# KyungMinJin/OTPose

Hardware: AMD Instinct MI355X
Metric: frames/sec at 384x288, 5-frame window, batch 16; heatmap max-abs delta vs ref (higher is better)
Workload: dtype f32 storage+accumulate / f16x3 split products; 1 GPU; BASELINE configs[1]: batch 16 x 5-frame x 384x288, HRNet-W48 + DCN warp + ConvVideoTransformer, fp32 forward (eval), seeded synthetic weights; clips_per_gpu=16, parallelism=dp1, outputs_finite=True

## Files before the change

include/otpose_hip.h:

```cpp
#ifndef OTPOSE_HIP_H
#define OTPOSE_HIP_H

#include <stddef.h>

#ifdef __cplusplus
extern "C" {
#endif

#define OTP_OK 0
#define OTP_ERR_BAD_ARG (-1)
#define OTP_ERR_UNSUPPORTED (-2)
#define OTP_ERR_LAUNCH (-3)
#define OTP_ERR_WORKSPACE (-4)

#define OTP_DTYPE_F32 0
#define OTP_DTYPE_F16 1
#define OTP_DTYPE_BF16 2
#define OTP_DTYPE_F64 3
#define OTP_DTYPE_I64 4

#define OTP_ACT_NONE 0
#define OTP_ACT_RELU 1
#define OTP_ACT_GELU 2

// ... 237 lines not shown
int otp_upsample_linear(const void* x, void* out, int B, int C, int T, int f, int out_ctot, int out_coff, void* stream);

int otp_mlp_fused_supported(int C, int HID, int T);
size_t otp_mlp_fused_weight_bytes(int C, int HID);
int otp_mlp_fused_pack(const void* w1, const void* b1, const void* w2, void* packed, int C, int HID, void* stream);
int otp_mlp_fused(const void* x, const void* packed, const void* scale, const void* shift, const void* res, void* out,
                  int B, int C, int HID, int T, void* stream);
int otp_ln_mlp_fused(const void* y, const void* ln_gamma, const void* ln_beta, float ln_eps, const void* packed,
                     const void* scale, const void* shift, void* out, int B, int C, int HID, int T, void* stream);

int otp_dense_x3_supported(int C, int T);
size_t otp_dense_x3_weight_bytes(int C);
int otp_dense_x3_pack(const void* w, const void* scale, const void* shift, void* packed, int C, void* stream);
int otp_dense_x3(const void* const* x, const void* const* packed, const void* const* res, void* const* out, int nprob, int B,
                 int C, int T, void* stream);
int otp_dense_x3_pack_bf16p(const void* w, const void* scale, const void* shift, void* packed, int C, void* stream);
int otp_dense_x3_bf16p(const void* const* x, const void* const* packed, const void* const* res, void* const* out, int nprob, int B,
                 int C, int T, void* stream);
int otp_qkv_front_x3(const void* x, const void* table, const void* packed_q, const void* packed_k, const void* packed_v,
                     void* q, void* k, void* v, int B, int C, int T, float eps, void* stream);

int otp_stem_conv_x3_supported(int B, int F, int H, int W, int Cout);
size_t otp_stem_conv_x3_weight_bytes(int Cout);
int otp_stem_conv_x3_pack(const void* w, const void* scale, const void* shift, void* packed, int Cout, void* stream);
int otp_stem_conv_x3(const void* in, const void* packed, void* out, int B, int F, int H, int W, int Cout, void* stream);

int otp_pointwise_x3_supported(int Cin, int Cout, int T);
size_t otp_pointwise_x3_weight_bytes(int Cin, int Cout);
int otp_pointwise_x3_pack(const void* w, const void* scale, const void* shift, void* packed, int Cin, int Cout, void* stream);
int otp_pointwise_x3(const void* x, const void* packed, const void* res, void* out, int B, int Cin, int Cout, int T, int x_ctot,
                     int x_coff, int res_ctot, int res_coff, int out_ctot, int out_coff, int relu, void* stream);
int otp_pointwise_x3_s8_supported(int Cin, int Cout, int T);
size_t otp_pointwise_x3_s8_weight_bytes(int Cin, int Cout);
int otp_pointwise_x3_s8_pack(const void* w, const void* scale, const void* shift, void* packed, int Cin, int Cout, void* stream);
int otp_pointwise_x3_s8(const void* x, const void* packed, void* out_s8, int B, int Cin, int Cout, int T, int x_ctot, int x_coff,
                        int relu, void* stream);
int otp_pointwise_x3_s8_res(const void* x, const void* packed, const void* res, void* out_s8, int B, int Cin, int Cout, int T,
                            int x_ctot, int x_coff, int r_ctot, int r_coff, int relu, void* stream);
int otp_pointwise_x3_pair_supported(int Cin, int Cmid, int Cout2, int T);
size_t otp_pointwise_x3_pair_weight_bytes(int Cin, int Cmid, int Cout2);
int otp_pointwise_x3_pair_pack(const void* w1, const void* scale1, const void* shift1, const void* w2, const void* scale2,
                               const void* shift2, void* packed, int Cin, int Cmid, int Cout2, void* stream);
int otp_pointwise_x3_pair(const void* x, const void* packed, const void* res, void* out, void* out_s8, int B, int Cin, int Cmid,
                          int Cout2, int T, int x_ctot, int x_coff, int res_ctot, int res_coff, int out_ctot, int out_coff,
                          int relu1, int relu2, void* stream);

int otp_mlp_x3_supported(int C, int HID, int T);
size_t otp_mlp_x3_weight_bytes(int C, int HID);
int otp_mlp_x3_pack(const void* w1, const void* b1, const void* w2, void* packed, int C, int HID, void* stream);
int otp_mlp_x3(const void* x, const void* packed, const void* scale, const void* shift, const void* res, void* out, int B,
               int C, int HID, int T, void* stream);
int otp_ln_mlp_x3(const void* y, const void* ln_gamma, const void* ln_beta, float ln_eps, const void* packed,
                  const void* scale, const void* shift, void* out, int B, int C, int HID, int T, void* stream);

int otp_flow_block_supported(int C, int hidden, int T);
size_t otp_flow_front_param_floats(int C);
size_t otp_flow_back_param_floats(int C, int hidden);
int otp_flow_front(const void* x, const void* params, void* q, void* k, void* v, int B, int C, int T, float eps, void* stream);
int otp_flow_back(const void* x, const void* att, const void* params, void* out, int B, int C, int hidden, int T, float eps,
                  void* stream);

int otp_dense_cc_supported(int C, int T);
size_t otp_dense_cc_weight_bytes(int C);
int otp_dense_cc_pack(const void* w, const void* scale, const void* shift, void* packed, int C, void* stream);
int otp_dense_cc(const void* const* x, const void* const* packed, const void* const* res, void* const* out, int nprob,
                 int B, int C, int T, void* stream);

size_t otp_qkv_front_table_bytes(int C);
int otp_qkv_front_pack_table(const void* dwq, const void* dwk, const void* dwv, const void* gq, const void* bq,
                             const void* gk, const void* bk, const void* gv, const void* bv, void* table, int C,
                             void* stream);
int otp_qkv_front(const void* x, const void* table, const void* packed_q, const void* packed_k, const void* packed_v,
                  void* q, void* k, void* v, int B, int C, int T, float eps, void* stream);

int otp_upsample_add(const void* low, const void* res, void* out, int N, int C, int Hl, int Wl, int f, int relu,
                     int low_ctot, int low_coff, int res_ctot, int res_coff, int out_ctot, int out_coff, void* stream);
int otp_upsample_add_multi(const void* const* lows, const int* factors, int nlow, const void* res, void* out, int N, int C,
                           int Hh, int Wh, int relu, int res_ctot, int res_coff, int out_ctot, int out_coff, void* stream);

int otp_chan_attn_set_split(int on);
int otp_chan_attn_splits(int BH, int T);
int otp_chan_attn_scores(const void* a, const void* b, void* slabs, int BH, int hs, int T, void* stream);
int otp_chan_attn_apply(const void* v, const void* M, void* out, int BH, int hs, int T, void* stream);
int otp_chan_attn_scores_bf16p(const void* a, const void* b, void* slabs, int BH, int hs, int T, void* stream);
int otp_chan_attn_apply_bf16p(const void* v, const void* M, void* out, int BH, int hs, int T, void* stream);
int otp_transpose_scale(const void* in, void* out, int batches, int R, int Cc, float scale, void* stream);
int otp_softmax_backward(const void* slabs, const void* P, void* dS, void* dST, void* PT, int BH, int hs, int NS,
                         void* stream);
int otp_softmax_backward_dropout(const void* slabs, const void* P, void* dS, void* dST, void* PT, int BH, int hs, int NS, float p,
                                 unsigned long long seed, void* stream);
int otp_ln_channel_backward(const void* x, const void* grad_y, const void* gamma, void* grad_x, void* dy_xhat, int B, int C,
                            int T, float eps, void* stream);
size_t otp_ln_channel_backward_workspace(int B, int C, int T);
int otp_ln_channel_backward_params(const void* x, const void* grad_y, const void* gamma, void* grad_x, void* grad_gamma,
                                   void* grad_beta, void* workspace, size_t workspace_bytes, int B, int C, int T, float eps,
                                   void* stream);
int otp_dwconv3_forward(const void* x, const void* w, void* y, int B, int C, int T, int stride, void* stream);
int otp_dwconv3_backward(const void* x, const void* w, const void* grad_y, void* grad_x, void* grad_w, int B, int C, int T,
                         int stride, void* stream);
int otp_gelu_forward(const void* x, void* y, size_t n, void* stream);
int otp_gelu_backward(const void* x, const void* grad_y, void* grad_x, size_t n, void* stream);
int otp_maxpool3s2_forward(const void* x, void* y, int rows, int T, void* stream);
int otp_maxpool3s2_backward(const void* x, const void* grad_y, void* grad_x, int rows, int T, void* stream);
int otp_upsample_linear_backward(const void* grad_out, void* grad_x, int B, int C, int T, int f, int out_ctot, int out_coff,
                                 void* stream);

int otp_upsample_add_backward(const void* grad_out, const void* out_relu, void* grad_res, void* grad_low, int planes, int Hl,
                              int Wl, int f, void* stream);

int otp_axpby(const void* x, void* y, float alpha, float beta, size_t n, void* stream);

int otp_heatmap_decode(const void* heatmaps, void* preds, void* maxvals, const void* center, const void* scale,
                       int N, int J, int H, int W, int refine, void* stream);

int otp_heatmap_flip_decode(const void* heatmaps, const int* perm, void* merged, void* preds, void* maxvals,
                            const void* center, const void* scale, int B, int J, int H, int W, int shift, void* stream);
int otp_clip_mirror_pair(const void* x, void* out, int B, int C, int H, int W, void* stream);

int otp_pck_accuracy(const void* pred_coords, const void* target_coords, void* acc, void* cnt, int N, int J, int H, int W,
                     float thr, void* stream);

size_t otp_grad_sumsq_scratch(void);
int otp_grad_sumsq(const void* grad, size_t n, void* acc_f64, void* stream);
int otp_adamw_step(void* param, const void* grad, void* exp_avg, void* exp_avg_sq, size_t n, float lr, float beta1,
                   float beta2, float eps, float weight_decay, int step, const void* gradnorm_sq_f64, float max_norm,
                   void* stream);
int otp_sgd_step(void* param, const void* grad, void* momentum_buf, size_t n, float lr, float momentum, float dampening,
                 float weight_decay, int nesterov, int first_step, const void* gradnorm_sq_f64, float max_norm, void* stream);

int otp_ema_update(void* ema, const void* src, size_t n, float decay, float one_minus_decay, void* stream);
size_t otp_ema_job_bytes(void);
int otp_ema_job(void* ema, const void* src, size_t count, int dtype, const void* prev_job_host, void* job_host);
int otp_ema_update_table(const void* jobs_device, int n_jobs, float decay, float one_minus_decay, void* stream);

int otp_frames_u8_to_clip(const void* frames_u8, void* out, int B, int F, int H, int W, float mean_r, float mean_g,
                          float mean_b, float std_r, float std_g, float std_b, void* stream);

int otp_crop_clips_u8(const void* pool_u8, int S, int Hp, int Wp, const void* frame_idx, const void* M, const void* flip,
                      void* out, int B, int F, int H, int W, float mean_r, float mean_g, float mean_b, float std_r,
                      float std_g, float std_b, void* stream);
int otp_crop_clips_blur_u8(const void* pool_u8, int S, int Hp, int Wp, const void* frame_idx, const void* M,
                           const void* flip, void* out, int B, int F, int H, int W, float mean_r, float mean_g,
                           float mean_b, float std_r, float std_g, float std_b, const void* blur, const void* blur_on,
                           void* stream);
int otp_crop_clips_pair_u8(const void* pool_u8, int S, int Hp, int Wp, const void* frame_idx, const void* M, void* out,
                           int B, int F, int H, int W, float mean_r, float mean_g, float mean_b, float std_r, float std_g,
                           float std_b, void* stream);
int otp_pose_plan(const void* boxes, const void* scores, const void* counts, const void* frame_number,
                  const void* num_frames, int S, int K, int detect_lo, int detect_hi, double min_score, double aspect_ratio,
                  double enlarge, int out_w, int out_h, int posetrack18, int max_persons, void* center, void* scale, void* M,
                  void* frame_idx, void* margin, void* box_score, void* person_slot, void* pr_off, void* total, void* stream);
int otp_pose_targets(const void* joints, const void* vis, const void* M, const void* gauss, void* target,
                     void* target_weight, int B, int J, int W, int H, int w, int h, int sigma3, void* stream);

size_t otp_loss_workspace(int B, int J);
int otp_loss_st_ohkw_grads(const void* s, const void* t, const void* g, const void* w, void* flags, void* result,
                           void* grad_s, void* grad_t, void* grad_g, void* workspace, size_t workspace_bytes, int B, int J,
                           int HW, int topk, int flags_given, void* stream);
int otp_loss_st_ohkw(const void* s, const void* t, const void* g, const void* w, void* flags,
                     void* result, void* grad_s, void* grad_t, void* workspace, size_t workspace_bytes,
                     int B, int J, int HW, int topk, int flags_given, void* stream);
int otp_loss_joints_mse(const void* o, const void* g, const void* w, void* result, void* grad_o, void* workspace,
                        size_t workspace_bytes, int B, int J, int HW, int topk, int ohkm, int effective_num_joints,
                        void* stream);


// ... 114 lines not shown
```

otpose_amd/csrc/transformer.hip:

```cpp
#include "x3.h"
#include <cstdlib>
#include <type_traits>

namespace {

template <int CREG>
__global__ __launch_bounds__(256) void ln_channel_kernel(const float* __restrict__ x, const float* __restrict__ gamma,
                                                          const float* __restrict__ beta, float* __restrict__ y,
                                                          int C, int T, float eps) {
    const int t = blockIdx.x * blockDim.x + threadIdx.x;
    if (t >= T) return;
    const size_t base = (size_t)blockIdx.y * C * T + t;
    const float inv_c = 1.f / (float)C;
    if (CREG > 0) {
        float v[CREG > 0 ? CREG : 1];
        float s = 0.f;
#pragma unroll
        for (int c = 0; c < CREG; ++c) {
            v[c] = c < C ? x[base + (size_t)c * T] : 0.f;
            s += v[c];
        }
        const float mu = s * inv_c;
        float q = 0.f;
#pragma unroll
// ... 429 lines not shown
    const float* vb = v + (size_t)bh * hs * T;
    const float* pb = P + (size_t)bh * HSP * HSP;
    {
        constexpr int NP4 = (HSP * HSP / 4 + 255) / 256, NV4 = (HSP * (TT / 4) + 255) / 256;
        const bool vecv = (T & 3) == 0 && (reinterpret_cast<uintptr_t>(v) & 15) == 0;
        otp_f32x4 rp[NP4], rv[NV4];
#pragma unroll
        for (int j = 0; j < NP4; ++j) {
            const int idx = tid + j * 256;
            rp[j] = idx < HSP * HSP / 4 ? reinterpret_cast<const otp_f32x4*>(pb)[idx] : (otp_f32x4){0.f, 0.f, 0.f, 0.f};
        }
#pragma unroll
        for (int j = 0; j < NV4; ++j) {
            const int idx = tid + j * 256;
            const int row = idx / (TT / 4), t = t0 + 4 * (idx - row * (TT / 4));
            otp_f32x4 a = {0.f, 0.f, 0.f, 0.f};
            if (row < hs && idx < HSP * (TT / 4)) {
                const float* vp = vb + (size_t)row * T + t;
                if (vecv && t + 3 < T) {
                    a = *reinterpret_cast<const otp_f32x4*>(vp);
                } else {
#pragma unroll
                    for (int e = 0; e < 4; ++e)
                        if (t + e < T) a[e] = vp[e];
                }
            }
            rv[j] = a;
        }
#pragma unroll
        for (int j = 0; j < NP4; ++j) {
            const int idx = tid + j * 256;
            if (idx < HSP * HSP / 4) {
                const int i = (4 * idx) / HSP, jj = 4 * idx - i * HSP;
#pragma unroll
                for (int e = 0; e < 4; ++e) pl[i * PS + jj + e] = rp[j][e];
            }
        }
#pragma unroll
        for (int j = 0; j < NV4; ++j) {
            const int idx = tid + j * 256;
            if (idx < HSP * (TT / 4)) {
                const int row = idx / (TT / 4), tt = 4 * (idx - row * (TT / 4));
                *reinterpret_cast<otp_f32x4*>(vl + row * VS + tt) = rv[j];
            }
        }
    }
    __syncthreads();
    const int r16 = lane & 15, kk = lane >> 4;
    otp_f32x4 acc[TB][NB];
#pragma unroll
    for (int tb = 0; tb < TB; ++tb)
#pragma unroll
        for (int ib = 0; ib < NB; ++ib) acc[tb][ib] = (otp_f32x4){0.f, 0.f, 0.f, 0.f};
    const float* va = vl + kk * VS + wave * (TT / 4) + r16;
    const float* pa = pl + r16 * PS + kk;
    for (int j0 = 0; j0 < HSP; j0 += 4) {
        float a[TB], b[NB];
#pragma unroll
        for (int tb = 0; tb < TB; ++tb) a[tb] = va[j0 * VS + tb * 16];
#pragma unroll
        for (int ib = 0; ib < NB; ++ib) b[ib] = pa[ib * 16 * PS + j0];
#pragma unroll
        for (int tb = 0; tb < TB; ++tb)
#pragma unroll
            for (int ib = 0; ib < NB; ++ib)
                acc[tb][ib] = __builtin_amdgcn_mfma_f32_16x16x4f32(a[tb], b[ib], acc[tb][ib], 0, 0, 0);
    }
    float* ob = out + (size_t)bh * T * hs;
#pragma unroll
    for (int tb = 0; tb < TB; ++tb)
#pragma unroll
        for (int r = 0; r < 4; ++r) {
            const int t = t0 + wave * (TT / 4) + tb * 16 + kk * 4 + r;
            if (t < T) {
#pragma unroll
                for (int ib = 0; ib < NB; ++ib) {
                    const int i = ib * 16 + r16;
                    if (i < hs) ob[(size_t)t * hs + i] = acc[tb][ib][r];
                }
            }
        }
}

constexpr size_t PVX_LDS = 138 * 1024;
constexpr int pvx_waves(int NB) { return NB <= 5 ? 8 : 4; }
constexpr size_t pvx_lds(int NB) {
    return NB <= 5 ? PVX_LDS : (size_t)(32 * pvx_waves(NB) + NB * 16) * (NB * 16 * 4 + 16) + 16;
}
template <typename P, int NB>
__global__ __launch_bounds__(64 * pvx_waves(NB), 2) void attn_pv_x3_kernel(const float* __restrict__ v, const float* __restrict__ M,
                                                                      float* __restrict__ out, int hs, int T, unsigned* rflag) {
    constexpr int PVX_WAVES = pvx_waves(NB), PVX_TH = 64 * PVX_WAVES, PVX_TT = 32 * PVX_WAVES;
    constexpr int HSP = NB * 16, KS = (HSP + 31) / 32, G = HSP / 8;
    constexpr int REC = HSP * 4 + 16;
    constexpr int NVI = (G * (PVX_TT / 4) + PVX_TH - 1) / PVX_TH;
    constexpr int NP4 = (HSP * HSP / 4 + PVX_TH - 1) / PVX_TH;
    extern __shared__ __attribute__((aligned(16))) unsigned char pvs[];
    unsigned char* vrec = pvs;
    unsigned char* prec = pvs + PVX_TT * REC;
    unsigned char* zrec = prec + HSP * REC;
    const int tid = threadIdx.x, lane = tid & 63, wave = tid >> 6;
    const int bh = blockIdx.x, t0 = blockIdx.y * PVX_TT;
    const float* vb = v + (size_t)bh * hs * T;
    const float* pb = M + (size_t)bh * HSP * HSP;
    if (tid < 4) reinterpret_cast<uint32_t*>(zrec)[tid] = 0u;
    {
        otp_f32x4 rp[NP4];
#pragma unroll
        for (int j = 0; j < NP4; ++j) {
            const int idx = tid + j * PVX_TH;
            rp[j] = idx < HSP * HSP / 4 ? reinterpret_cast<const otp_f32x4*>(pb)[idx] : (otp_f32x4){0.f, 0.f, 0.f, 0.f};
        }
#pragma unroll
        for (int j = 0; j < NP4; ++j) {
            const int idx = tid + j * PVX_TH;
            if (idx < HSP * HSP / 4) {
                const int i = (4 * idx) / HSP, jj = 4 * idx - i * HSP;
                unsigned long long h, l;
                otp_x3_split4<P>(rp[j], h, l);
                *reinterpret_cast<unsigned long long*>(prec + i * REC + jj * 2) = h;
                *reinterpret_cast<unsigned long long*>(prec + i * REC + HSP * 2 + jj * 2) = l;
            }
        }
    }
    const bool vecv = (T & 3) == 0 && (reinterpret_cast<uintptr_t>(v) & 15) == 0;
#pragma unroll
    for (int it = 0; it < NVI; ++it) {
        const int idx = tid + it * PVX_TH;
        const int g = idx / (PVX_TT / 4), f4 = idx - g * (PVX_TT / 4);
        const int t = t0 + 4 * f4;
        otp_f32x4 x[8];
#pragma unroll
        for (int e = 0; e < 8; ++e) {
            const int row = 8 * g + e;
            otp_f32x4 a = {0.f, 0.f, 0.f, 0.f};
            if (idx < G * (PVX_TT / 4) && row < hs) {
                const float* vp = vb + (size_t)row * T + t;
                if (vecv && t + 3 < T) {
                    a = *reinterpret_cast<const otp_f32x4*>(vp);
                } else {
#pragma unroll
                    for (int c = 0; c < 4; ++c)
                        if (t + c < T) a[c] = vp[c];
                }
            }
            x[e] = a;
        }
        if (idx < G * (PVX_TT / 4)) {
#pragma unroll
            for (int c = 0; c < 4; ++c) {
                unsigned long long h0, l0, h1, l1;
                otp_x3_split4<P>((otp_f32x4){x[0][c], x[1][c], x[2][c], x[3][c]}, h0, l0);
                otp_x3_split4<P>((otp_f32x4){x[4][c], x[5][c], x[6][c], x[7][c]}, h1, l1);
                unsigned char* r = vrec + (4 * f4 + c) * REC + g * 16;
                *reinterpret_cast<unsigned long long*>(r) = h0;
                *reinterpret_cast<unsigned long long*>(r + 8) = h1;
                *reinterpret_cast<unsigned long long*>(r + HSP * 2) = l0;
                *reinterpret_cast<unsigned long long*>(r + HSP * 2 + 8) = l1;
            }
        }
    }
    __syncthreads();
    const int r16 = lane & 15, kk = lane >> 4;
    otp_f32x4 acc[2][NB];
#pragma unroll
    for (int mt = 0; mt < 2; ++mt)
#pragma unroll
        for (int nt = 0; nt < NB; ++nt) acc[mt][nt] = (otp_f32x4){0.f, 0.f, 0.f, 0.f};
#pragma unroll
    for (int ks = 0; ks < KS; ++ks) {
        const int kg = 4 * ks + kk;
        const bool kv = kg < G;
        typename P::x8 ah[2], al[2];
#pragma unroll
        for (int mt = 0; mt < 2; ++mt) {
            const unsigned char* a = kv ? vrec + ((wave * 2 + mt) * 16 + r16) * REC + kg * 16 : zrec;
            ah[mt] = *reinterpret_cast<const typename P::x8*>(a);
            al[mt] = *reinterpret_cast<const typename P::x8*>(kv ? a + HSP * 2 : zrec);
        }
#pragma unroll
        for (int nt = 0; nt < NB; ++nt) {
            const unsigned char* b = kv ? prec + (nt * 16 + r16) * REC + kg * 16 : zrec;
            const typename P::x8 b_h = *reinterpret_cast<const typename P::x8*>(b);
            const typename P::x8 b_l = *reinterpret_cast<const typename P::x8*>(kv ? b + HSP * 2 : zrec);
#pragma unroll
            for (int mt = 0; mt < 2; ++mt) {
                acc[mt][nt] = P::mfma(al[mt], b_h, acc[mt][nt]);
                acc[mt][nt] = P::mfma(ah[mt], b_l, acc[mt][nt]);
                acc[mt][nt] = P::mfma(ah[mt], b_h, acc[mt][nt]);
            }
        }
    }
    {
        bool bad = false;
#pragma unroll
        for (int mt = 0; mt < 2; ++mt)
#pragma unroll
            for (int nt = 0; nt < NB; ++nt)
#pragma unroll
                for (int r = 0; r < 4; ++r) bad |= otp_out_of_range<P>(acc[mt][nt][r]);
        otp_range_report(rflag, bad, OTP_RANGE_ATTN);
    }
    float* ob = out + (size_t)bh * T * hs;
#pragma unroll
    for (int mt = 0; mt < 2; ++mt)
#pragma unroll
        for (int r = 0; r < 4; ++r) {
            const int t = t0 + (wave * 2 + mt) * 16 + kk * 4 + r;
            if (t < T) {
#pragma unroll
                for (int nt = 0; nt < NB; ++nt) {
                    const int i = nt * 16 + r16;
                    if (i < hs) ob[(size_t)t * hs + i] = acc[mt][nt][r];
                }
            }
        }
}

__global__ void upsample_linear_kernel(const float* __restrict__ x, float* __restrict__ out, int C, int T, int f,
                                       int out_ctot, int out_coff) {
    const int To = T * f;
    const int to = blockIdx.x * blockDim.x + threadIdx.x;
    if (to >= To) return;
    const int c = blockIdx.y % C, b = blockIdx.y / C;
    const float* xr = x + ((size_t)b * C + c) * T;
    float r;
    if (f == 1) {
        r = xr[to];
    } else {
        float src = ((float)to + 0.5f) * (1.f / (float)f) - 0.5f;
        src = src < 0.f ? 0.f : src;
        int i0 = (int)src;
        int i1 = i0 + (i0 < T - 1 ? 1 : 0);
        float l1 = src - (float)i0, l0 = 1.f - l1;
        r = l0 * xr[i0] + l1 * xr[i1];
    }
    out[((size_t)b * out_ctot + out_coff + c) * To + to] = r;
}

__global__ void upsample_linear4_kernel(const float* __restrict__ x, float* __restrict__ out, int C, int T, int f,
                                        int out_ctot, int out_coff) {
    const int To = T * f;
    const int t4 = (blockIdx.x * blockDim.x + threadIdx.x) * 4;
    if (t4 >= To) return;
    const int c = blockIdx.y % C, b = blockIdx.y / C;
    const float* xr = x + ((size_t)b * C + c) * T;
    otp_f32x4 r;
    if (f == 1) {
        r = *reinterpret_cast<const otp_f32x4*>(xr + t4);
    } else {
        const float inv = 1.f / (float)f;
#pragma unroll
        for (int k = 0; k < 4; ++k) {
            float src = ((float)(t4 + k) + 0.5f) * inv - 0.5f;
            src = src < 0.f ? 0.f : src;
            const int i0 = (int)src;
            const int i1 = i0 + (i0 < T - 1 ? 1 : 0);
            const float l1 = src - (float)i0, l0 = 1.f - l1;
            r[k] = l0 * xr[i0] + l1 * xr[i1];
        }
    }
    *reinterpret_cast<otp_f32x4*>(out + ((size_t)b * out_ctot + out_coff + c) * To + t4) = r;
}

}

extern "C" int otp_ln_channel(const void* x, const void* gamma, const void* beta, void* y, void* pool, int B,
                              int C, int T, float eps, void* stream) {
    if (!x || !gamma || !beta || !y || B <= 0 || C <= 0 || T <= 0) return OTP_ERR_BAD_ARG;
    auto st = static_cast<hipStream_t>(stream);
    auto xf = static_cast<const float*>(x);
    auto gf = static_cast<const float*>(gamma);
    auto bf = static_cast<const float*>(beta);
    auto yf = static_cast<float*>(y);
    dim3 grid(otp_ceil_div(T, 256), B);
    if (C <= 17) hipLaunchKernelGGL(ln_channel_kernel<17>, grid, dim3(256), 0, st, xf, gf, bf, yf, C, T, eps);
    else if (C <= 136)
        hipLaunchKernelGGL(ln_channel_split_kernel<34>, dim3(otp_ceil_div(T, 64), B), dim3(256), 0, st, xf, gf, bf, yf, C, T, eps);
    else if (C <= 204)
        hipLaunchKernelGGL(ln_channel_split_kernel<51>, dim3(otp_ceil_div(T, 64), B), dim3(256), 0, st, xf, gf, bf, yf, C, T, eps);
    else hipLaunchKernelGGL(ln_channel_kernel<0>, grid, dim3(256), 0, st, xf, gf, bf, yf, C, T, eps);
    if (pool) {
        int To = (T + 2 - 3) / 2 + 1;
        hipLaunchKernelGGL(maxpool3s2_kernel, dim3(otp_ceil_div(To, 256), B * C), dim3(256), 0, st, xf,
                           static_cast<float*>(pool), T, To);
    }
    return otp_launch_status();
}

extern "C" int otp_dwconv_ln3(const void* x, const void* dwq, const void* dwk, const void* dwv, const void* gq,
                              const void* bq, const void* gk, const void* bk, const void* gv, const void* bv,
                              void* q, void* k, void* v, int B, int C, int T, int stride, float eps, void* stream) {
    if (!x || !dwq || !dwk || !dwv || !gq || !bq || !gk || !bk || !gv || !bv || !q || !k || !v) return OTP_ERR_BAD_ARG;
    if (B <= 0 || C <= 0 || T <= 0 || stride <= 0) return OTP_ERR_BAD_ARG;
    const int To = (T + 2 - 3) / stride + 1;
    auto f = [](const void* p) { return static_cast<const float*>(p); };
    auto st = static_cast<hipStream_t>(stream);
#define OTP_DW_ARGS f(x), f(dwq), f(dwk), f(dwv), f(gq), f(bq), f(gk), f(bk), f(gv), f(bv), static_cast<float*>(q), \
                    static_cast<float*>(k), static_cast<float*>(v), C, T, To, stride, eps
    if (C <= 4 * 5)
        hipLaunchKernelGGL(dwconv_ln3_kernel<5>, dim3(otp_ceil_div(To, 64), B), dim3(256), 0, st, OTP_DW_ARGS);
    else if (C <= 4 * 34)
        hipLaunchKernelGGL(dwconv_ln3_kernel<34>, dim3(otp_ceil_div(To, 64), B), dim3(256), 0, st, OTP_DW_ARGS);
    else if (C <= 4 * 51)
        hipLaunchKernelGGL(dwconv_ln3_kernel<51>, dim3(otp_ceil_div(To, 64), B), dim3(256), 0, st, OTP_DW_ARGS);
    else
        hipLaunchKernelGGL(dwconv_ln3_generic_kernel, dim3(otp_ceil_div(To, 256), B), dim3(256), 0, st, OTP_DW_ARGS);
#undef OTP_DW_ARGS
    return otp_launch_status();
}
namespace {
std::atomic<int> g_attn_split{1};

int attn_splits(int BH, int T) {
    int ns = 1;
    while (BH * ns < 768 && T / (ns * 2) >= 2 * ATT_TC) ns *= 2;
    return ns;
}

template <typename F>
void with_nb(int hs, F f) {
    switch ((hs + 15) / 16) {
        case 1: f(std::integral_constant<int, 1>{}); break;
        case 2: f(std::integral_constant<int, 2>{}); break;
        case 3: f(std::integral_constant<int, 3>{}); break;
        case 4: f(std::integral_constant<int, 4>{}); break;
        case 5: f(std::integral_constant<int, 5>{}); break;
        case 6: f(std::integral_constant<int, 6>{}); break;
        default: f(std::integral_constant<int, 7>{}); break;
    }
}

template <typename P>
void launch_scores(const float* a, const float* b, float* slabs, int BH, int hs, int T, int NS, int chunk, hipStream_t st) {
    const bool split = g_attn_split.load(std::memory_order_relaxed);
    with_nb(hs, [&](auto nb) {
        constexpr int NB = decltype(nb)::value;
        if (split) {
            auto kern = attn_scores_x3_kernel<P, NB>;
            const size_t lds = (size_t)4 * NB * 16 * SX_PITCH;
            OTP_ALLOW_BIG_LDS(kern, lds);
            hipLaunchKernelGGL(kern, dim3(BH, NS), dim3(256), lds, st, a, b, slabs, hs, T, chunk);
        } else {
            hipLaunchKernelGGL(attn_scores_kernel<NB>, dim3(BH, NS), dim3(256), 0, st, a, b, slabs, hs, T, chunk);
        }
    });
}

template <int NB>
void launch_pv_f32(const float* v, const float* M, float* out, int BH, int hs, int T, hipStream_t st) {
    constexpr int HSP = NB * 16, TT = pv_tt(NB);
    const size_t lds = ((size_t)HSP * (HSP + 2) + (size_t)HSP * (TT + 16)) * sizeof(float);
    auto kern = attn_pv_kernel<NB>;
    OTP_ALLOW_BIG_LDS(kern, lds);
    hipLaunchKernelGGL(kern, dim3(BH, otp_ceil_div(T, TT)), dim3(256), lds, st, v, M, out, hs, T);
}

template <typename P>
void launch_apply(const float* v, const float* M, float* out, int BH, int hs, int T, hipStream_t st) {
    const bool split = g_attn_split.load(std::memory_order_relaxed);
    with_nb(hs, [&](auto nb) {
        constexpr int NB = decltype(nb)::value;
        if (split) {
            auto kern = attn_pv_x3_kernel<P, NB>;
            const size_t lds = pvx_lds(NB);
            OTP_ALLOW_BIG_LDS(kern, lds);
            hipLaunchKernelGGL(kern, dim3(BH, otp_ceil_div(T, 32 * pvx_waves(NB))), dim3(64 * pvx_waves(NB)), lds, st, v, M, out, hs,
                               T, otp_range_word());
        } else {
            launch_pv_f32<NB>(v, M, out, BH, hs, T, st);
        }
    });
}

template <typename P>
int scores_entry(const void* a, const void* b, void* slabs, int BH, int hs, int T, void* stream) {
    if (!a || !b || !slabs || BH <= 0 || hs <= 0 || T <= 0) return OTP_ERR_BAD_ARG;
    if (hs > 7 * 16) return OTP_ERR_UNSUPPORTED;
    const int NS = attn_splits(BH, T);
    const int chunk = otp_ceil_div(otp_ceil_div(T, NS), ATT_TC) * ATT_TC;
    launch_scores<P>(static_cast<const float*>(a), static_cast<const float*>(b), static_cast<float*>(slabs), BH, hs, T, NS, chunk,
                     static_cast<hipStream_t>(stream));
    return otp_launch_status();
}

template <typename P>
int apply_entry(const void* v, const void* M, void* out, int BH, int hs, int T, void* stream) {
    if (!v || !M || !out || BH <= 0 || hs <= 0 || T <= 0) return OTP_ERR_BAD_ARG;
    if (hs > 7 * 16) return OTP_ERR_UNSUPPORTED;
    launch_apply<P>(static_cast<const float*>(v), static_cast<const float*>(M), static_cast<float*>(out), BH, hs, T,
                    static_cast<hipStream_t>(stream));
    return otp_launch_status();
}
}

extern "C" size_t otp_chan_attn_workspace(int B, int C, int T, int n_head) {
    if (B <= 0 || C <= 0 || T <= 0 || n_head <= 0 || C % n_head) return 0;
    const int hs = C / n_head, HSP = (hs + 15) & ~15;
    const size_t BH = (size_t)B * n_head;
    return (BH * attn_splits((int)BH, T) + BH) * HSP * HSP * sizeof(float);
}

extern "C" int otp_chan_attn(const void* q, const void* k, const void* v, void* out, void* workspace,
                             size_t workspace_bytes, int B, int C, int T, int n_head, float scale, void* stream) {
    if (!q || !k || !v || !out || !workspace || B <= 0 || C <= 0 || T <= 0 || n_head <= 0) return OTP_ERR_BAD_ARG;
    if (C % n_head) return OTP_ERR_BAD_ARG;
    const int hs = C / n_head, HSP = (hs + 15) & ~15;
    if (HSP > 7 * 16) return OTP_ERR_UNSUPPORTED;
    if (workspace_bytes < otp_chan_attn_workspace(B, C, T, n_head)) return OTP_ERR_WORKSPACE;
    const int BH = B * n_head, NS = attn_splits(BH, T);
    const int chunk = otp_ceil_div(otp_ceil_div(T, NS), ATT_TC) * ATT_TC;
    auto st = static_cast<hipStream_t>(stream);
    float* slabs = static_cast<float*>(workspace);
    float* P = slabs + (size_t)BH * NS * HSP * HSP;
    launch_scores<otp_half_pieces>(static_cast<const float*>(q), static_cast<const float*>(k), slabs, BH, hs, T, NS, chunk, st);
    hipLaunchKernelGGL(attn_softmax_kernel, dim3(BH, otp_ceil_div(HSP, 4)), dim3(256), 0, st, slabs, P, hs, HSP, NS, scale);
    launch_apply<otp_half_pieces>(static_cast<const float*>(v), P, static_cast<float*>(out), BH, hs, T, st);
    return otp_launch_status();
}

extern "C" size_t otp_chan_attn_dropout_workspace(int B, int C, int T, int n_head) {
    const size_t base = otp_chan_attn_workspace(B, C, T, n_head);
    if (!base) return 0;
    const int hs = C / n_head, HSP = (hs + 15) & ~15;
    return base + (size_t)B * n_head * HSP * HSP * sizeof(float);
}

extern "C" int otp_chan_attn_dropout(const void* q, const void* k, const void* v, void* out, void* workspace, size_t workspace_bytes,
                                     int B, int C, int T, int n_head, float scale, float p, unsigned long long seed, void* stream) {
    if (!q || !k || !v || !out || !workspace || B <= 0 || C <= 0 || T <= 0 || n_head <= 0 || !otp_attn_drop_rate_ok(p))
        return OTP_ERR_BAD_ARG;
    if (C % n_head) return OTP_ERR_BAD_ARG;
    const otp_attn_drop drop = otp_attn_drop_make(p, seed);
    if (!drop.thr) return otp_chan_attn(q, k, v, out, workspace, workspace_bytes, B, C, T, n_head, scale, stream);
    const int hs = C / n_head, HSP = (hs + 15) & ~15;
    if (HSP > 7 * 16) return OTP_ERR_UNSUPPORTED;
    if (workspace_bytes < otp_chan_attn_dropout_workspace(B, C, T, n_head)) return OTP_ERR_WORKSPACE;
    const int BH = B * n_head, NS = attn_splits(BH, T);
    const int chunk = otp_ceil_div(otp_ceil_div(T, NS), ATT_TC) * ATT_TC;
    auto st = static_cast<hipStream_t>(stream);
    float* slabs = static_cast<float*>(workspace);
    float* P = slabs + (size_t)BH * NS * HSP * HSP;
    float* PM = P + (size_t)BH * HSP * HSP;
    launch_scores<otp_half_pieces>(static_cast<const float*>(q), static_cast<const float*>(k), slabs, BH, hs, T, NS, chunk, st);
    hipLaunchKernelGGL(attn_softmax_drop_kernel, dim3(BH, otp_ceil_div(HSP, 4)), dim3(256), 0, st, slabs, P, PM, hs, HSP, NS, scale,
                       drop);
    launch_apply<otp_half_pieces>(static_cast<const float*>(v), PM, static_cast<float*>(out), BH, hs, T, st);
    return otp_launch_status();
}

extern "C" int otp_chan_attn_set_split(int on) {
    g_attn_split.store(on ? 1 : 0, std::memory_order_relaxed);
    return OTP_OK;
}

extern "C" int otp_chan_attn_splits(int BH, int T) { return (BH > 0 && T > 0) ? attn_splits(BH, T) : 0; }

extern "C" int otp_chan_attn_scores(const void* a, const void* b, void* slabs, int BH, int hs, int T, void* stream) {
    return scores_entry<otp_half_pieces>(a, b, slabs, BH, hs, T, stream);
}
extern "C" int otp_chan_attn_scores_bf16p(const void* a, const void* b, void* slabs, int BH, int hs, int T, void* stream) {
    return scores_entry<otp_bf16_pieces>(a, b, slabs, BH, hs, T, stream);
}

extern "C" int otp_chan_attn_apply(const void* v, const void* M, void* out, int BH, int hs, int T, void* stream) {
    return apply_entry<otp_half_pieces>(v, M, out, BH, hs, T, stream);
}
extern "C" int otp_chan_attn_apply_bf16p(const void* v, const void* M, void* out, int BH, int hs, int T, void* stream) {
    return apply_entry<otp_bf16_pieces>(v, M, out, BH, hs, T, stream);
}

extern "C" int otp_maxpool3s2_forward(const void* x, void* y, int rows, int T, void* stream) {
    if (!x || !y || rows <= 0 || T <= 0) return OTP_ERR_BAD_ARG;
    const int To = (T + 2 - 3) / 2 + 1;
    hipLaunchKernelGGL(maxpool3s2_kernel, dim3(otp_ceil_div(To, 256), rows), dim3(256), 0, static_cast<hipStream_t>(stream),
                       static_cast<const float*>(x), static_cast<float*>(y), T, To);
    return otp_launch_status();
}

extern "C" int otp_upsample_linear(const void* x, void* out, int B, int C, int T, int f, int out_ctot, int out_coff,
                                   void* stream) {
    if (!x || !out || B <= 0 || C <= 0 || T <= 0 || f <= 0 || out_ctot < out_coff + C) return OTP_ERR_BAD_ARG;
    const bool vec = (T * f) % 4 == 0 && (f > 1 || T % 4 == 0) &&
                     ((reinterpret_cast<uintptr_t>(x) | reinterpret_cast<uintptr_t>(out)) & 15) == 0;
    if (vec)
        hipLaunchKernelGGL(upsample_linear4_kernel, dim3(otp_ceil_div(T * f / 4, 256), B * C), dim3(256), 0,
                           static_cast<hipStream_t>(stream), static_cast<const float*>(x), static_cast<float*>(out), C, T,
                           f, out_ctot, out_coff);
    else
        hipLaunchKernelGGL(upsample_linear_kernel, dim3(otp_ceil_div(T * f, 256), B * C), dim3(256), 0,
                           static_cast<hipStream_t>(stream), static_cast<const float*>(x), static_cast<float*>(out), C, T,
                           f, out_ctot, out_coff);
    return otp_launch_status();
}
```

Before: 3295 frames/s.

## Make attention PV kernel persistent with double-buffered V tiles

Rewrites the x3-split attention apply (P·V) kernel as a persistent kernel. The grid is sized from the CU count, and each workgroup loops over a contiguous range of token tiles. The next V tile's global loads are issued before the MFMA work on the current tile, then written into a second LDS buffer. The per-block P-matrix split is amortised across many tiles, and loads and stores now go through buffer resources with OOB masking. The aim is to hide V-load latency and cut repeated P staging, at the cost of larger LDS use, possibly lower occupancy, and one new host query of the device CU count.

New measurement: 3300 frames/s (median of 2 runs). About the same (+0.1%).

```diff
diff --git a/include/otpose_hip.h b/include/otpose_hip.h
--- a/include/otpose_hip.h
+++ b/include/otpose_hip.h
@@ -343,6 +343,8 @@
 int otp_chan_attn_splits(int BH, int T);
 int otp_chan_attn_scores(const void* a, const void* b, void* slabs, int BH, int hs, int T, void* stream);
 int otp_chan_attn_apply(const void* v, const void* M, void* out, int BH, int hs, int T, void* stream);
+int otp_chan_attn_pv_tile(int hs);
+int otp_chan_attn_pv_workgroups(int BH, int hs);
 int otp_chan_attn_scores_bf16p(const void* a, const void* b, void* slabs, int BH, int hs, int T, void* stream);
 int otp_chan_attn_apply_bf16p(const void* v, const void* M, void* out, int BH, int hs, int T, void* stream);
 int otp_transpose_scale(const void* in, void* out, int batches, int R, int Cc, float scale, void* stream);
diff --git a/otpose_amd/csrc/transformer.hip b/otpose_amd/csrc/transformer.hip
--- a/otpose_amd/csrc/transformer.hip
+++ b/otpose_amd/csrc/transformer.hip
@@ -535,38 +535,78 @@
         }
 }
 
-constexpr size_t PVX_LDS = 138 * 1024;
-constexpr int pvx_waves(int NB) { return NB <= 5 ? 8 : 4; }
-constexpr size_t pvx_lds(int NB) {
-    return NB <= 5 ? PVX_LDS : (size_t)(32 * pvx_waves(NB) + NB * 16) * (NB * 16 * 4 + 16) + 16;
-}
-template <typename P, int NB>
-__global__ __launch_bounds__(64 * pvx_waves(NB), 2) void attn_pv_x3_kernel(const float* __restrict__ v, const float* __restrict__ M,
-                                                                      float* __restrict__ out, int hs, int T, unsigned* rflag) {
-    constexpr int PVX_WAVES = pvx_waves(NB), PVX_TH = 64 * PVX_WAVES, PVX_TT = 32 * PVX_WAVES;
+constexpr int pvx_mt(int NB) { return NB <= 2 ? 4 : NB == 3 ? 2 : 1; }
+constexpr int pvx_tt(int NB) { return 64 * pvx_mt(NB); }
+constexpr size_t pvx_lds(int NB) { return (size_t)(2 * pvx_tt(NB) + NB * 16 + 1) * (NB * 16 * 4 + 16) + 16 + 256 * 8; }
+constexpr int pvx_per_cu(int NB) { return 2 * pvx_lds(NB) <= OTP_LDS_LIMIT ? 2 : 1; }
+template <typename P, int NB, bool VEC>
+__global__ __launch_bounds__(256, 2) void attn_pv_x3_kernel(const float* __restrict__ v, const float* __restrict__ M,
+                                                             float* __restrict__ out, int hs, int T, unsigned* rflag) {
+    constexpr int MT = pvx_mt(NB), PVX_TT = pvx_tt(NB);
     constexpr int HSP = NB * 16, KS = (HSP + 31) / 32, G = HSP / 8;
     constexpr int REC = HSP * 4 + 16;
-    constexpr int NVI = (G * (PVX_TT / 4) + PVX_TH - 1) / PVX_TH;
-    constexpr int NP4 = (HSP * HSP / 4 + PVX_TH - 1) / PVX_TH;
+    constexpr int NP4 = (HSP * HSP / 4 + 255) / 256;
+    static_assert(G * (PVX_TT / 4) <= 256, "one v item (8 rows x 4 tokens) per thread");
     extern __shared__ __attribute__((aligned(16))) unsigned char pvs[];
-    unsigned char* vrec = pvs;
-    unsigned char* prec = pvs + PVX_TT * REC;
+    unsigned char* prec = pvs + 2 * PVX_TT * REC;
     unsigned char* zrec = prec + HSP * REC;
+    unsigned char* spare = zrec + 16;
     const int tid = threadIdx.x, lane = tid & 63, wave = tid >> 6;
-    const int bh = blockIdx.x, t0 = blockIdx.y * PVX_TT;
+    const int bh = blockIdx.x;
+    const int ntiles = (T + PVX_TT - 1) / PVX_TT, W = gridDim.y, w = blockIdx.y;
+    const int per = ntiles / W, rem = ntiles - per * W;
+    const int first = w * per + min(w, rem), count = per + (w < rem ? 1 : 0);
+    if (count == 0) return;
     const float* vb = v + (size_t)bh * hs * T;
     const float* pb = M + (size_t)bh * HSP * HSP;
+    const bool loader = tid < G * (PVX_TT / 4);
+    const int g = tid / (PVX_TT / 4), f4 = tid - g * (PVX_TT / 4);
+    const otp_rsrc rv = make_rsrc32(vb, (unsigned)hs * (unsigned)T * 4u);
+    otp_f32x4 x[8];
+    auto load_tile = [&](int tile) __attribute__((always_inline)) {
+        const int t = tile * PVX_TT + 4 * f4;
+        if constexpr (VEC) {
+#pragma unroll
+            for (int e = 0; e < 8; ++e) {
+                const int row = 8 * g + e;
+                x[e] = bload4(rv, (loader && row < hs && t < T) ? (int)(((unsigned)row * (unsigned)T + (unsigned)t) * 4u) : OTP_OOB);
+            }
+        } else {
+#pragma unroll
+            for (int e = 0; e < 8; ++e) {
+                const int row = 8 * g + e;
+#pragma unroll
+                for (int c = 0; c < 4; ++c)
+                    x[e][c] = bload(rv, (loader && row < hs && t + c < T) ? (int)(((unsigned)row * (unsigned)T + (unsigned)(t + c)) * 4u)
+                                                                         : OTP_OOB, 0);
+            }
+        }
+    };
+    auto write_tile = [&](unsigned char* vrec) __attribute__((always_inline)) {
+#pragma unroll
+        for (int c = 0; c < 4; ++c) {
+            unsigned long long h0, l0, h1, l1;
+            otp_x3_split4<P>((otp_f32x4){x[0][c], x[1][c], x[2][c], x[3][c]}, h0, l0);
+            otp_x3_split4<P>((otp_f32x4){x[4][c], x[5][c], x[6][c], x[7][c]}, h1, l1);
+            unsigned char* r = loader ? vrec + (4 * f4 + c) * REC + g * 16 : spare + tid * 8;
+            *reinterpret_cast<unsigned long long*>(r) = h0;
+            *reinterpret_cast<unsigned long long*>(r + 8) = h1;
+            *reinterpret_cast<unsigned long long*>(r + HSP * 2) = l0;
+            *reinterpret_cast<unsigned long long*>(r + HSP * 2 + 8) = l1;
+        }
+    };
+    load_tile(first);
     if (tid < 4) reinterpret_cast<uint32_t*>(zrec)[tid] = 0u;
     {
         otp_f32x4 rp[NP4];
 #pragma unroll
         for (int j = 0; j < NP4; ++j) {
-            const int idx = tid + j * PVX_TH;
+            const int idx = tid + j * 256;
             rp[j] = idx < HSP * HSP / 4 ? reinterpret_cast<const otp_f32x4*>(pb)[idx] : (otp_f32x4){0.f, 0.f, 0.f, 0.f};
         }
 #pragma unroll
         for (int j = 0; j < NP4; ++j) {
-            const int idx = tid + j * PVX_TH;
+            const int idx = tid + j * 256;
             if (idx < HSP * HSP / 4) {
                 const int i = (4 * idx) / HSP, jj = 4 * idx - i * HSP;
                 unsigned long long h, l;
@@ -576,98 +616,65 @@
             }
         }
     }
-    const bool vecv = (T & 3) == 0 && (reinterpret_cast<uintptr_t>(v) & 15) == 0;
-#pragma unroll
-    for (int it = 0; it < NVI; ++it) {
-        const int idx = tid + it * PVX_TH;
-        const int g = idx / (PVX_TT / 4), f4 = idx - g * (PVX_TT / 4);
-        const int t = t0 + 4 * f4;
-        otp_f32x4 x[8];
-#pragma unroll
-        for (int e = 0; e < 8; ++e) {
-            const int row = 8 * g + e;
-            otp_f32x4 a = {0.f, 0.f, 0.f, 0.f};
-            if (idx < G * (PVX_TT / 4) && row < hs) {
-                const float* vp = vb + (size_t)row * T + t;
-                if (vecv && t + 3 < T) {
-                    a = *reinterpret_cast<const otp_f32x4*>(vp);
-                } else {
-#pragma unroll
-                    for (int c = 0; c < 4; ++c)
-                        if (t + c < T) a[c] = vp[c];
+    write_tile(pvs);
+    const int r16 = lane & 15, kk = lane >> 4;
+    const otp_rsrc ro = make_rsrc32(out + (size_t)bh * T * hs, (unsigned)hs * (unsigned)T * 4u);
+    bool bad = false;
+    for (int it = 0; it < count; ++it) {
+        __syncthreads();
+        const unsigned char* vrec = pvs + (it & 1) * (PVX_TT * REC);
+        load_tile(it + 1 < count ? first + it + 1 : ntiles);
+        __builtin_amdgcn_sched_barrier(0);
+        otp_f32x4 acc[MT][NB];
+#pragma unroll
+        for (int mt = 0; mt < MT; ++mt)
+#pragma unroll
+            for (int nt = 0; nt < NB; ++nt) acc[mt][nt] = (otp_f32x4){0.f, 0.f, 0.f, 0.f};
+#pragma unroll
+        for (int ks = 0; ks < KS; ++ks) {
+            const int kg = 4 * ks + kk;
+            const bool kv = kg < G;
+            typename P::x8 ah[MT], al[MT];
+#pragma unroll
+            for (int mt = 0; mt < MT; ++mt) {
+                const unsigned char* a = kv ? vrec + ((wave * MT + mt) * 16 + r16) * REC + kg * 16 : zrec;
+                ah[mt] = *reinterpret_cast<const typename P::x8*>(a);
+                al[mt] = *reinterpret_cast<const typename P::x8*>(kv ? a + HSP * 2 : zrec);
+            }
+#pragma unroll
+            for (int nt = 0; nt < NB; ++nt) {
+                const unsigned char* b = kv ? prec + (nt * 16 + r16) * REC + kg * 16 : zrec;
+                const typename P::x8 b_h = *reinterpret_cast<const typename P::x8*>(b);
+                const typename P::x8 b_l = *reinterpret_cast<const typename P::x8*>(kv ? b + HSP * 2 : zrec);
+#pragma unroll
+                for (int mt = 0; mt < MT; ++mt) {
+                    acc[mt][nt] = P::mfma(al[mt], b_h, acc[mt][nt]);
+                    acc[mt][nt] = P::mfma(ah[mt], b_l, acc[mt][nt]);
+                    acc[mt][nt] = P::mfma(ah[mt], b_h, acc[mt][nt]);
                 }
             }
-            x[e] = a;
-        }
-        if (idx < G * (PVX_TT / 4)) {
-#pragma unroll
-            for (int c = 0; c < 4; ++c) {
-                unsigned long long h0, l0, h1, l1;
-                otp_x3_split4<P>((otp_f32x4){x[0][c], x[1][c], x[2][c], x[3][c]}, h0, l0);
-                otp_x3_split4<P>((otp_f32x4){x[4][c], x[5][c], x[6][c], x[7][c]}, h1, l1);
-                unsigned char* r = vrec + (4 * f4 + c) * REC + g * 16;
-                *reinterpret_cast<unsigned long long*>(r) = h0;
-                *reinterpret_cast<unsigned long long*>(r + 8) = h1;
-                *reinterpret_cast<unsigned long long*>(r + HSP * 2) = l0;
-                *reinterpret_cast<unsigned long long*>(r + HSP * 2 + 8) = l1;
-            }
-        }
-    }
-    __syncthreads();
-    const int r16 = lane & 15, kk = lane >> 4;
-    otp_f32x4 acc[2][NB];
-#pragma unroll
-    for (int mt = 0; mt < 2; ++mt)
-#pragma unroll
-        for (int nt = 0; nt < NB; ++nt) acc[mt][nt] = (otp_f32x4){0.f, 0.f, 0.f, 0.f};
-#pragma unroll
-    for (int ks = 0; ks < KS; ++ks) {
-        const int kg = 4 * ks + kk;
-        const bool kv = kg < G;
-        typename P::x8 ah[2], al[2];
-#pragma unroll
-        for (int mt = 0; mt < 2; ++mt) {
-            const unsigned char* a = kv ? vrec + ((wave * 2 + mt) * 16 + r16) * REC + kg * 16 : zrec;
-            ah[mt] = *reinterpret_cast<const typename P::x8*>(a);
-            al[mt] = *reinterpret_cast<const typename P::x8*>(kv ? a + HSP * 2 : zrec);
-        }
-#pragma unroll
-        for (int nt = 0; nt < NB; ++nt) {
-            const unsigned char* b = kv ? prec + (nt * 16 + r16) * REC + kg * 16 : zrec;
-            const typename P::x8 b_h = *reinterpret_cast<const typename P::x8*>(b);
-            const typename P::x8 b_l = *reinterpret_cast<const typename P::x8*>(kv ? b + HSP * 2 : zrec);
-#pragma unroll
-            for (int mt = 0; mt < 2; ++mt) {
-                acc[mt][nt] = P::mfma(al[mt], b_h, acc[mt][nt]);
-                acc[mt][nt] = P::mfma(ah[mt], b_l, acc[mt][nt]);
-                acc[mt][nt] = P::mfma(ah[mt], b_h, acc[mt][nt]);
-            }
-        }
-    }
-    {
-        bool bad = false;
-#pragma unroll
-        for (int mt = 0; mt < 2; ++mt)
+        }
+        write_tile(pvs + ((it + 1) & 1) * (PVX_TT * REC));
+#pragma unroll
+        for (int mt = 0; mt < MT; ++mt)
 #pragma unroll
             for (int nt = 0; nt < NB; ++nt)
 #pragma unroll
                 for (int r = 0; r < 4; ++r) bad |= otp_out_of_range<P>(acc[mt][nt][r]);
-        otp_range_report(rflag, bad, OTP_RANGE_ATTN);
-    }
-    float* ob = out + (size_t)bh * T * hs;
-#pragma unroll
-    for (int mt = 0; mt < 2; ++mt)
-#pragma unroll
-        for (int r = 0; r < 4; ++r) {
-            const int t = t0 + (wave * 2 + mt) * 16 + kk * 4 + r;
-            if (t < T) {
+        const int t0 = (first + it) * PVX_TT;
+#pragma unroll
+        for (int mt = 0; mt < MT; ++mt)
+#pragma unroll
+            for (int r = 0; r < 4; ++r) {
+                const int t = t0 + (wave * MT + mt) * 16 + kk * 4 + r;
 #pragma unroll
                 for (int nt = 0; nt < NB; ++nt) {
                     const int i = nt * 16 + r16;
-                    if (i < hs) ob[(size_t)t * hs + i] = acc[mt][nt][r];
+                    bstore(acc[mt][nt][r], ro, (i < hs && t < T) ? (int)(((unsigned)t * (unsigned)hs + (unsigned)i) * 4u) : OTP_OOB, 0);
                 }
             }
-        }
+    }
+    otp_range_report(rflag, bad, OTP_RANGE_ATTN);
 }
 
 __global__ void upsample_linear_kernel(const float* __restrict__ x, float* __restrict__ out, int C, int T, int f,
@@ -765,6 +772,8 @@
 namespace {
 std::atomic<int> g_attn_split{1};
 
+bool attn_slab_ok(int hs, int T) { return (size_t)hs * T < ((size_t)1 << 30); }
+
 int attn_splits(int BH, int T) {
     int ns = 1;
     while (BH * ns < 768 && T / (ns * 2) >= 2 * ATT_TC) ns *= 2;
@@ -782,6 +791,26 @@
         case 6: f(std::integral_constant<int, 6>{}); break;
         default: f(std::integral_constant<int, 7>{}); break;
     }
+}
+
+int device_cus() {
+    static std::atomic<int> cus[OTP_MAX_DEVICES];
+    int dev = 0;
+    if (hipGetDevice(&dev) != hipSuccess) return 0;
+    std::atomic<int>& c = cus[dev & (OTP_MAX_DEVICES - 1)];
+    int n = c.load(std::memory_order_relaxed);
+    if (n <= 0) {
+        if (hipDeviceGetAttribute(&n, hipDeviceAttributeMultiprocessorCount, dev) != hipSuccess || n <= 0) return 0;
+        c.store(n, std::memory_order_relaxed);
+    }
+    return n;
+}
+
+int pv_workgroups(int BH, int NB) {
+    int per_cu = 1;
+    with_nb(NB * 16, [&](auto nb) { per_cu = pvx_per_cu(decltype(nb)::value); });
+    const int w = device_cus() * per_cu / BH;
+    return w > 0 ? w : 1;
 }
 
 template <typename P>
@@ -815,11 +844,17 @@
     with_nb(hs, [&](auto nb) {
         constexpr int NB = decltype(nb)::value;
         if (split) {
-            auto kern = attn_pv_x3_kernel<P, NB>;
             const size_t lds = pvx_lds(NB);
-            OTP_ALLOW_BIG_LDS(kern, lds);
-            hipLaunchKernelGGL(kern, dim3(BH, otp_ceil_div(T, 32 * pvx_waves(NB))), dim3(64 * pvx_waves(NB)), lds, st, v, M, out, hs,
-                               T, otp_range_word());
+            const dim3 grid(BH, pv_workgroups(BH, NB));
+            if ((T & 3) == 0 && (reinterpret_cast<uintptr_t>(v) & 15) == 0) {
+                auto kern = attn_pv_x3_kernel<P, NB, true>;
+                OTP_ALLOW_BIG_LDS(kern, lds);
+                hipLaunchKernelGGL(kern, grid, dim3(256), lds, st, v, M, out, hs, T, otp_range_word());
+            } else {
+                auto kern = attn_pv_x3_kernel<P, NB, false>;
+                OTP_ALLOW_BIG_LDS(kern, lds);
+                hipLaunchKernelGGL(kern, grid, dim3(256), lds, st, v, M, out, hs, T, otp_range_word());
+            }
         } else {
             launch_pv_f32<NB>(v, M, out, BH, hs, T, st);
         }
@@ -840,7 +875,7 @@
 template <typename P>
 int apply_entry(const void* v, const void* M, void* out, int BH, int hs, int T, void* stream) {
     if (!v || !M || !out || BH <= 0 || hs <= 0 || T <= 0) return OTP_ERR_BAD_ARG;
-    if (hs > 7 * 16) return OTP_ERR_UNSUPPORTED;
+    if (hs > 7 * 16 || !attn_slab_ok(hs, T)) return OTP_ERR_UNSUPPORTED;
     launch_apply<P>(static_cast<const float*>(v), static_cast<const float*>(M), static_cast<float*>(out), BH, hs, T,
                     static_cast<hipStream_t>(stream));
     return otp_launch_status();
@@ -859,7 +894,7 @@
     if (!q || !k || !v || !out || !workspace || B <= 0 || C <= 0 || T <= 0 || n_head <= 0) return OTP_ERR_BAD_ARG;
     if (C % n_head) return OTP_ERR_BAD_ARG;
     const int hs = C / n_head, HSP = (hs + 15) & ~15;
-    if (HSP > 7 * 16) return OTP_ERR_UNSUPPORTED;
+    if (HSP > 7 * 16 || !attn_slab_ok(hs, T)) return OTP_ERR_UNSUPPORTED;
     if (workspace_bytes < otp_chan_attn_workspace(B, C, T, n_head)) return OTP_ERR_WORKSPACE;
     const int BH = B * n_head, NS = attn_splits(BH, T);
     const int chunk = otp_ceil_div(otp_ceil_div(T, NS), ATT_TC) * ATT_TC;
@@ -887,7 +922,7 @@
     const otp_attn_drop drop = otp_attn_drop_make(p, seed);
     if (!drop.thr) return otp_chan_attn(q, k, v, out, workspace, workspace_bytes, B, C, T, n_head, scale, stream);
     const int hs = C / n_head, HSP = (hs + 15) & ~15;
-    if (HSP > 7 * 16) return OTP_ERR_UNSUPPORTED;
+    if (HSP > 7 * 16 || !attn_slab_ok(hs, T)) return OTP_ERR_UNSUPPORTED;
     if (workspace_bytes < otp_chan_attn_dropout_workspace(B, C, T, n_head)) return OTP_ERR_WORKSPACE;
     const int BH = B * n_head, NS = attn_splits(BH, T);
     const int chunk = otp_ceil_div(otp_ceil_div(T, NS), ATT_TC) * ATT_TC;
@@ -908,6 +943,16 @@
 }
 
 extern "C" int otp_chan_attn_splits(int BH, int T) { return (BH > 0 && T > 0) ? attn_splits(BH, T) : 0; }
+
+extern "C" int otp_chan_attn_pv_tile(int hs) {
+    if (hs <= 0 || hs > 7 * 16) return 0;
+    int tt = 0;
+    with_nb(hs, [&](auto nb) { tt = pvx_tt(decltype(nb)::value); });
+    return tt;
+}
+extern "C" int otp_chan_attn_pv_workgroups(int BH, int hs) {
+    return (BH > 0 && hs > 0 && hs <= 7 * 16) ? pv_workgroups(BH, (hs + 15) / 16) : 0;
+}
 
 extern "C" int otp_chan_attn_scores(const void* a, const void* b, void* slabs, int BH, int hs, int T, void* stream) {
     return scores_entry<otp_half_pieces>(a, b, slabs, BH, hs, T, stream);
```
